# ahmetumutdurmus/zaremba

Measured on NVIDIA H100. Metric: tokens/sec (and valid perplexity) Large-LSTM 1500h at 1/2/4/8 H100 vs ref CPU, higher is better.
Workload: dtype f16 operands, f32 accumulate/state

## Files before the change

### zaremba_b200/csrc/gemm_tc.cu

```cuda
#include <stdlib.h>
#include <string.h>

#include "kernels.h"
#include "tc_common.cuh"
#include "tc_host.h"

namespace zrb {

using namespace tc;

constexpr int GBM = 128, GBK = 64;
constexpr int kASubBytes = GBM * GBK * 2;
constexpr int kEpiWarps = 8;
constexpr int kGemmThreads = 3 * 128;
template <int GBN> struct GemmCfg {
    static constexpr int kStages = GBN == 256 ? 4 : 6;
    static constexpr int kABytes = kASubBytes;
    static constexpr int kBBytes = GBN * GBK * 2;
    static constexpr int kSmem = kStages * (kABytes + kBBytes) + 1024  + 256 ;
};

struct GemmArgs {
    int M, N, K;
    float alpha;
    const float* bias;
    const float* bias2;
    float* C;
    int64_t ldc;
    int accumulate;
    int tiles_m, tiles_n;
    int splits;
    float* sumsq_out;
    float* C2;
    float* sumsq_out2;
    const __half* a_tiled;
    const __half* b_tiled;
    int a_nt128, b_nt128;
    int pdl_trigger;
    int pdl_tail;
    int epi_direct;
};

template <int GBN> constexpr int kStagger = GemmCfg<GBN>::kStages - 1;
constexpr int kStaggerBar = 1;

template <bool A_MN, bool B_MN, int GBN>
__global__ void __launch_bounds__(kGemmThreads, 1)
gemm_f16_tc_kernel(const __grid_constant__ CUtensorMap tma_a, const __grid_constant__ CUtensorMap tma_b,
                   const __grid_constant__ CUtensorMap tma_b2, GemmArgs p) {
    using Cfg = GemmCfg<GBN>;
    constexpr int kStages = Cfg::kStages;
    constexpr int kABytes = Cfg::kABytes;
    constexpr int kBBytes = Cfg::kBBytes;
    extern __shared__ uint8_t smem_raw[];
    uint8_t* smem = (uint8_t*)(((uintptr_t)smem_raw + 1023) & ~(uintptr_t)1023);
    uint8_t* sA = smem;
    uint8_t* sB = smem + kStages * kABytes;
    uint64_t* bars = (uint64_t*)(smem + kStages * (kABytes + kBBytes));
    uint64_t* full = bars;
    uint64_t* empty = bars + kStages;

    const int warp = __shfl_sync(0xffffffffu, (int)(threadIdx.x >> 5), 0);
    const int lane = threadIdx.x & 31;
    const int num_tiles = p.tiles_m * p.tiles_n;
    const int num_kb = (p.K + GBK - 1) / GBK;
    const bool dual = p.C2 != nullptr;
    const int num_work = dual ? 2 * num_tiles : num_tiles * p.splits;
    const int kb_per = (num_kb + p.splits - 1) / p.splits;

    if (threadIdx.x == 0) {
        if (p.pdl_trigger) asm volatile("griddepcontrol.launch_dependents;" ::: "memory");
        tma_prefetch_desc(&tma_a);
        tma_prefetch_desc(&tma_b);
        if (dual) tma_prefetch_desc(&tma_b2);
        for (int i = 0; i < kStages; ++i) { mbar_init(&full[i], 1); mbar_init(&empty[i], kEpiWarps); }
        fence_mbar_init();
    }
    __syncthreads();

    if (warp < 4) {
        asm volatile("setmaxnreg.dec.sync.aligned.u32 40;" ::: "memory");
        if (warp == 0 && lane == 0) {
            int s = 0; uint32_t ph = 0;
            for (int w = blockIdx.x; w < num_work; w += gridDim.x) {
                const int tile = w % num_tiles, sp = dual ? 0 : w / num_tiles;
                const int kb0 = sp * kb_per, kb1 = min(num_kb, kb0 + kb_per);
                const CUtensorMap* tmb = (dual && w >= num_tiles) ? &tma_b2 : &tma_b;
                const int m0 = (tile % p.tiles_m) * GBM, n0 = (tile / p.tiles_m) * GBN;
                for (int kb = kb0; kb < kb1; ++kb) {
                    mbar_wait(&empty[s], ph ^ 1);
                    mbar_expect_tx(&full[s], kABytes + kBBytes);
                    uint8_t* a = sA + s * kABytes;
                    uint8_t* b = sB + s * kBBytes;
                    if (!A_MN && p.a_tiled) {
                        bulk_load_1d(a, p.a_tiled + ((size_t)kb * p.a_nt128 + (m0 >> 7)) * (128 * GBK), kASubBytes, &full[s]);
                    } else if (!A_MN) {
                        tma_load_2d(a, &tma_a, &full[s], kb * GBK, m0);
                    } else {
                        tma_load_2d(a, &tma_a, &full[s], m0, kb * GBK);
                        tma_load_2d(a + kASubBytes / 2, &tma_a, &full[s], m0 + 64, kb * GBK);
                    }
                    if (!B_MN && p.b_tiled) {
                        bulk_load_1d(b, p.b_tiled + ((size_t)kb * p.b_nt128 + (n0 >> 7)) * (128 * GBK), kBBytes, &full[s]);
                    } else if (!B_MN) {
                        tma_load_2d(b, tmb, &full[s], kb * GBK, n0);
                    } else {
#pragma unroll
                        for (int j = 0; j < GBN / 64; ++j)
                            tma_load_2d(b + j * (GBK * 128), tmb, &full[s], n0 + 64 * j, kb * GBK);
                    }
                    if (++s == kStages) { s = 0; ph ^= 1; }
                }
            }
        }
    } else {
        asm volatile("setmaxnreg.inc.sync.aligned.u32 232;" ::: "memory");
        const int cw = warp - 4;
        const int wg = cw >> 2;
        const int t = (int)threadIdx.x - 128 * (1 + wg);
        int s = 0; uint32_t ph = 0;
        float acc[GBN / 2];
        bool started_wg1 = p.epi_direct || wg == 1;
        if (!p.epi_direct && wg == 1) asm volatile("bar.sync %0, 256;" :: "n"(kStaggerBar) : "memory");
        int kb_issued = 0;
        const bool pair_store = !p.epi_direct && !p.accumulate && (p.ldc & 1) == 0 && ((uintptr_t)p.C & 7) == 0 &&
                                ((uintptr_t)p.C2 & 7) == 0;
        for (int w = blockIdx.x; w < num_work; w += gridDim.x) {
            const int tile = w % num_tiles, split = dual ? 0 : w / num_tiles;
            const int kb0 = split * kb_per, kb1 = min(num_kb, kb0 + kb_per);
            float* const Cout = (dual && w >= num_tiles) ? p.C2 : p.C;
            float* const ssq = (dual && w >= num_tiles) ? p.sumsq_out2 : p.sumsq_out;
            const int m0 = (tile % p.tiles_m) * GBM + 64 * wg, n0 = (tile / p.tiles_m) * GBN;
#pragma unroll
            for (int i = 0; i < GBN / 2; ++i) acc[i] = 0.f;
            wgmma_fence();
            wgmma_fence_acc(acc);
            int prev = -1;
            for (int kb = kb0; kb < kb1; ++kb) {
                mbar_wait(&full[s], ph);
                const uint32_t a_addr = smem_u32(sA + s * kABytes) + wg * (kASubBytes / 2);
                const uint32_t b_addr = smem_u32(sB + s * kBBytes);
#pragma unroll
                for (int k = 0; k < GBK / 16; ++k) {
                    const uint64_t da = A_MN ? make_smem_desc(a_addr + k * 2048, GBK * 128, 1024, kSwizzle128B)
                                             : make_smem_desc(a_addr + k * 32, 16, 1024, kSwizzle128B);
                    const uint64_t db = B_MN ? make_smem_desc(b_addr + k * 2048, GBK * 128, 1024, kSwizzle128B)
                                             : make_smem_desc(b_addr + k * 32, 16, 1024, kSwizzle128B);
                    Wgmma<GBN, A_MN ? 1 : 0, B_MN ? 1 : 0>::mma(acc, da, db, 1u);
                }
                wgmma_commit();
                if (!started_wg1 && ++kb_issued == kStagger<GBN>) {
                    asm volatile("bar.arrive %0, 256;" :: "n"(kStaggerBar) : "memory");
                    started_wg1 = true;
                }
                wgmma_wait<1>();
                if (prev >= 0) {
                    __syncwarp();
                    if (lane == 0) mbar_arrive(&empty[prev]);
                }
                prev = s;
                if (++s == kStages) { s = 0; ph ^= 1; }
            }
            if (!started_wg1) {
                asm volatile("bar.arrive %0, 256;" :: "n"(kStaggerBar) : "memory");
                started_wg1 = true;
            }
            wgmma_wait<0>();
            wgmma_fence_acc(acc);
            if (prev >= 0) {
                __syncwarp();
                if (lane == 0) mbar_arrive(&empty[prev]);
            }
            const bool add_bias = p.bias != nullptr && split == 0;
            float ss = 0.f;
#pragma unroll
            for (int h = 0; h < 2; ++h) {
                const int row = m0 + wgmma_row(t, h);
                if (row >= p.M) continue;
                float* const crow = Cout + (int64_t)row * p.ldc;
#pragma unroll
                for (int c8 = 0; c8 < GBN / 8; ++c8) {
                    const int col0 = n0 + wgmma_col(t, c8);
                    if (pair_store && col0 + 1 < p.N) {
                        const float bv0 = add_bias ? p.bias[col0] + (p.bias2 ? p.bias2[col0] : 0.f) : 0.f;
                        const float bv1 = add_bias ? p.bias[col0 + 1] + (p.bias2 ? p.bias2[col0 + 1] : 0.f) : 0.f;
                        const float o0 = p.alpha * acc[4 * c8 + 2 * h] + bv0;
                        const float o1 = p.alpha * acc[4 * c8 + 2 * h + 1] + bv1;
                        if (p.splits > 1) {
                            atomicAdd(reinterpret_cast<float2*>(crow + col0), make_float2(o0, o1));
                        } else {
                            *reinterpret_cast<float2*>(crow + col0) = make_float2(o0, o1);
                            ss += o0 * o0;
                            ss += o1 * o1;
                        }
                        continue;
                    }
#pragma unroll
                    for (int e = 0; e < 2; ++e) {
                        const int col = n0 + wgmma_col(t, c8) + e;
                        if (col >= p.N) continue;
                        const float bv = add_bias ? p.bias[col] + (p.bias2 ? p.bias2[col] : 0.f) : 0.f;
                        const float o = p.alpha * acc[4 * c8 + 2 * h + e] + bv;
                        if (p.splits > 1) {
                            atomicAdd(crow + col, o);
                        } else if (p.accumulate) {
                            crow[col] += o;
                        } else {
                            crow[col] = o;
                            ss += o * o;
                        }
                    }
                }
            }
            if (ssq) {
                ss = warp_sum(ss);
                if (lane == 0) ssq[tile * 8 + cw] = ss;
            }
        }
        if (!started_wg1) asm volatile("bar.arrive %0, 256;" :: "n"(kStaggerBar) : "memory");
    }
    if (p.pdl_tail && blockIdx.x == 0 && threadIdx.x == 0) asm volatile("griddepcontrol.wait;" ::: "memory");
}

namespace {

typedef CUresult (*EncodeTiledFn)(CUtensorMap*, CUtensorMapDataType, cuuint32_t, void*, const cuuint64_t*,
                                  const cuuint64_t*, const cuuint32_t*, const cuuint32_t*, CUtensorMapInterleave,
                                  CUtensorMapSwizzle, CUtensorMapL2promotion, CUtensorMapFloatOOBfill);

EncodeTiledFn get_encode() {
    static EncodeTiledFn fn = nullptr;
    static bool tried = false;
    if (!tried) {
        tried = true;
        void* p = nullptr;
        cudaDriverEntryPointQueryResult q;
        if (cudaGetDriverEntryPoint("cuTensorMapEncodeTiled", &p, cudaEnableDefault, &q) == cudaSuccess &&
            q == cudaDriverEntryPointSuccess)
            fn = (EncodeTiledFn)p;
    }
    return fn;
}

int g_num_sms = 0;
bool g_attr_set[64][8] = {};

}

int tc_num_sms() {
    if (!g_num_sms) {
        int dev = 0;
        cudaGetDevice(&dev);
        cudaDeviceGetAttribute(&g_num_sms, cudaDevAttrMultiProcessorCount, dev);
        if (g_num_sms <= 0) g_num_sms = 132;
    }
    return g_num_sms;
}

int tc_make_tmap_f16(CUtensorMap* m, const void* ptr, uint64_t inner, uint64_t outer, uint64_t ld, uint32_t box_inner,
                     uint32_t box_outer, int swizzle128) {
    EncodeTiledFn enc = get_encode();
    if (!enc) {
        set_error("cuTensorMapEncodeTiled not available from the driver");
        return ZRB_E_CUDA;
    }
    ZRB_REQUIRE((ld * 2) % 16 == 0 && (((uintptr_t)ptr) & 15) == 0, "TMA operand needs 16-byte aligned base and pitch");
    cuuint64_t dims[2] = {inner, outer};
    cuuint64_t strides[1] = {ld * 2};
    cuuint32_t box[2] = {box_inner, box_outer};
    cuuint32_t estr[2] = {1, 1};
    CUresult r = enc(m, CU_TENSOR_MAP_DATA_TYPE_FLOAT16, 2, const_cast<void*>(ptr), dims, strides, box, estr,
                     CU_TENSOR_MAP_INTERLEAVE_NONE, swizzle128 ? CU_TENSOR_MAP_SWIZZLE_128B : CU_TENSOR_MAP_SWIZZLE_NONE,
                     CU_TENSOR_MAP_L2_PROMOTION_L2_256B, CU_TENSOR_MAP_FLOAT_OOB_FILL_NONE);
    if (r != CUDA_SUCCESS) {
        set_error("cuTensorMapEncodeTiled failed (%d) inner=%llu outer=%llu ld=%llu", (int)r,
                  (unsigned long long)inner, (unsigned long long)outer, (unsigned long long)ld);
        return ZRB_E_CUDA;
    }
    return ZRB_OK;
}

template <bool A_MN, bool B_MN, int GBN>
static int launch_gemm(const CUtensorMap& ta, const CUtensorMap& tb, const CUtensorMap& tb2, const GemmArgs& a,
                       cudaStream_t s) {
    auto kern = gemm_f16_tc_kernel<A_MN, B_MN, GBN>;
    const int idx = (A_MN ? 2 : 0) + (B_MN ? 1 : 0) + (GBN == 256 ? 4 : 0);
    int dev = 0;
    cudaGetDevice(&dev);
    dev &= 63;
    if (!g_attr_set[dev][idx]) {
        ZRB_CUDA(cudaFuncSetAttribute(kern, cudaFuncAttributeMaxDynamicSharedMemorySize, GemmCfg<GBN>::kSmem));
        g_attr_set[dev][idx] = true;
    }
    int grid = a.tiles_m * a.tiles_n * (a.C2 ? 2 : a.splits);
    if (grid > tc_num_sms()) grid = tc_num_sms();
    if (a.pdl_tail) {
        grid = a.tiles_m * a.tiles_n * (a.C2 ? 2 : a.splits);
        cudaLaunchConfig_t cfg = {};
        cfg.gridDim = dim3(grid); cfg.blockDim = dim3(kGemmThreads);
        cfg.dynamicSmemBytes = GemmCfg<GBN>::kSmem; cfg.stream = s;
        cudaLaunchAttribute at[1];
        at[0].id = cudaLaunchAttributeProgrammaticStreamSerialization;
        at[0].val.programmaticStreamSerializationAllowed = 1;
        cfg.attrs = at; cfg.numAttrs = 1;
        ZRB_CUDA(cudaLaunchKernelEx(&cfg, kern, ta, tb, tb2, a));
        count_launch();
        return ZRB_OK;
    }
    kern<<<grid, kGemmThreads, GemmCfg<GBN>::kSmem, s>>>(ta, tb, tb2, a);
    ZRB_KERNEL_CHECK();
    return ZRB_OK;
}

template <int GBN>
static int dispatch_gemm(const CUtensorMap& ta, const CUtensorMap& tb, const CUtensorMap& tb2, const GemmArgs& a,
                         int a_mn, int b_mn, cudaStream_t s) {
    if (!a_mn && !b_mn) return launch_gemm<false, false, GBN>(ta, tb, tb2, a, s);
    if (!a_mn && b_mn) return launch_gemm<false, true, GBN>(ta, tb, tb2, a, s);
    if (a_mn && !b_mn) return launch_gemm<true, false, GBN>(ta, tb, tb2, a, s);
    return launch_gemm<true, true, GBN>(ta, tb, tb2, a, s);
}

struct TileChoice { int bn, tiles_m, tiles_n, splits; };
static TileChoice choose_tiles(int M, int N, int num_kb, bool can_split, bool retile = false) {
    const int nsm = tc_num_sms();
    TileChoice c;
    c.tiles_m = cdiv(M, GBM);
    const int t256 = c.tiles_m * cdiv(N, 256);
    if (can_split && t256 * 2 <= nsm && t256 * 2 >= (nsm * 4) / 10 && num_kb / 2 >= 8) {
        c.bn = 256; c.tiles_n = cdiv(N, 256); c.splits = 2;
        return c;
    }
    c.bn = (t256 >= (nsm * 9) / 10) ? 256 : 128;
    static const int force_bn = [] { const char* e = getenv("ZRB_GEMM_BN"); return e ? atoi(e) : 0; }();
    if (force_bn == 128 || force_bn == 256) c.bn = force_bn;
    else if (retile && c.bn == 256 && cdiv(t256, nsm) * 2 > cdiv(c.tiles_m * cdiv(N, 128), nsm) &&
             c.tiles_m * cdiv(N, 128) * 2 > nsm)
        c.bn = 128;
    c.tiles_n = cdiv(N, c.bn);
    c.splits = (can_split && c.tiles_m * c.tiles_n * 2 <= nsm && num_kb >= 8) ? 2 : 1;
    return c;
}

int gemm_f16_tc_sumsq_slots(int M, int N, int K) {
    TileChoice c = choose_tiles(M, N, cdiv(K, GBK), false);
    return c.tiles_m * c.tiles_n * kEpiWarps;
}

int gemm_f16_tc(const __half* A, int64_t lda, int a_mn, const __half* B, int64_t ldb, int b_mn, float* C, int64_t ldc,
                int M, int N, int K, float alpha, const float* bias, int accumulate, cudaStream_t s, float* sumsq_out,
                const float* bias2, bool pdl, const __half* B2, float* C2, float* sumsq_out2, const __half* A_tiled,
                int a_nt128, const __half* B_tiled, int b_nt128) {
    if (M <= 0 || N <= 0) return ZRB_OK;
    ZRB_REQUIRE(!B2 == !C2, "dual launch needs both B2 and C2");
    ZRB_REQUIRE(!bias2 || bias, "bias2 needs bias");
    ZRB_REQUIRE(!sumsq_out || !accumulate, "sumsq_out needs a plain store epilogue");
    ZRB_REQUIRE(K > 0, "gemm_f16_tc needs K > 0");
    const char* epi = getenv("ZRB_GEMM_EPI");
    const bool direct = epi && strcmp(epi, "direct") == 0;
    const TileChoice tc = choose_tiles(M, N, cdiv(K, GBK), !sumsq_out && ldc == N && !C2 && !accumulate,
                                       !direct && !sumsq_out && !C2 && !accumulate);
    const int bn = tc.bn;
    CUtensorMap ta, tb;
    if (!a_mn) ZRB_TRY(tc_make_tmap_f16(&ta, A, K, M, lda, GBK, GBM, 1));
    else       ZRB_TRY(tc_make_tmap_f16(&ta, A, M, K, lda, 64, GBK, 1));
    if (!b_mn) ZRB_TRY(tc_make_tmap_f16(&tb, B, K, N, ldb, GBK, bn, 1));
    else       ZRB_TRY(tc_make_tmap_f16(&tb, B, N, K, ldb, 64, GBK, 1));
    CUtensorMap tb2 = tb;
    if (B2) {
        if (!b_mn) ZRB_TRY(tc_make_tmap_f16(&tb2, B2, K, N, ldb, GBK, bn, 1));
        else       ZRB_TRY(tc_make_tmap_f16(&tb2, B2, N, K, ldb, 64, GBK, 1));
    }
    GemmArgs a;
    a.M = M; a.N = N; a.K = K; a.alpha = alpha; a.bias = bias; a.C = C; a.ldc = ldc; a.accumulate = accumulate;
    a.tiles_m = tc.tiles_m; a.tiles_n = tc.tiles_n;
    a.splits = tc.splits;
    a.sumsq_out = sumsq_out;
    a.bias2 = bias2;
    a.C2 = C2; a.sumsq_out2 = sumsq_out2;
    a.a_tiled = a_mn ? nullptr : A_tiled; a.a_nt128 = a_nt128; a.b_tiled = b_mn ? nullptr : B_tiled; a.b_nt128 = b_nt128;
    a.pdl_tail = (pdl && a.splits == 1) ? 1 : 0;
    a.pdl_trigger = (rec_pdl_enabled() && !a.pdl_tail) ? 1 : 0;
    a.epi_direct = direct ? 1 : 0;
    if (a.splits > 1 && !accumulate) ZRB_CUDA(cudaMemsetAsync(C, 0, (size_t)M * N * sizeof(float), s));
    return bn == 256 ? dispatch_gemm<256>(ta, tb, tb2, a, a_mn, b_mn, s) : dispatch_gemm<128>(ta, tb, tb2, a, a_mn, b_mn, s);
}

}

extern "C" int zrb_gemm_f16_tiled(const void* A, int64_t lda, const void* B, int64_t ldb, const void* A_tiled, int32_t a_nt128,
                                  const void* B_tiled, int32_t b_nt128, float* C, int64_t ldc, int32_t M, int32_t N, int32_t K,
                                  float alpha, void* stream) {
    ZRB_REQUIRE(A && B && C, "null argument");
    return zrb::gemm_f16_tc((const __half*)A, lda, 0, (const __half*)B, ldb, 0, C, ldc, M, N, K, alpha, nullptr, 0,
                            (cudaStream_t)stream, nullptr, nullptr, false, nullptr, nullptr, nullptr, (const __half*)A_tiled,
                            a_nt128, (const __half*)B_tiled, b_nt128);
}

extern "C" int zrb_gemm_f16(const void* A, int64_t lda, int32_t a_mn_major, const void* B, int64_t ldb,
                            int32_t b_mn_major, float* C, int64_t ldc, int32_t M, int32_t N, int32_t K, float alpha,
                            const float* bias, int32_t accumulate, void* stream) {
    ZRB_REQUIRE(A && B && C, "null argument");
    return zrb::gemm_f16_tc((const __half*)A, lda, a_mn_major, (const __half*)B, ldb, b_mn_major, C, ldc, M, N, K,
                            alpha, bias, accumulate, (cudaStream_t)stream, nullptr, nullptr, false, nullptr, nullptr, nullptr, nullptr, 0, nullptr, 0);
}
```

Measured before the change: 385,500.

## Add ping-pong consumer warpgroup schedule for large 128x128 GEMMs

```diff
diff --git a/zaremba_b200/csrc/gemm_tc.cu b/zaremba_b200/csrc/gemm_tc.cu
--- a/zaremba_b200/csrc/gemm_tc.cu
+++ b/zaremba_b200/csrc/gemm_tc.cu
@@ -41,13 +41,69 @@
     int epi_direct;
 };
 
-template <int GBN> constexpr int kStagger = GemmCfg<GBN>::kStages - 1;
+template <int GBN> constexpr int kStagger = GBN == 256 ? 1 : 2;
 constexpr int kStaggerBar = 1;
-
-template <bool A_MN, bool B_MN, int GBN>
+constexpr int kTurnBar = 1;
+__device__ __forceinline__ void turn_sync(int g) {
+    if (g == 0) asm volatile("bar.sync %0, 256;" :: "n"(kTurnBar) : "memory");
+    else        asm volatile("bar.sync %0, 256;" :: "n"(kTurnBar + 1) : "memory");
+}
+__device__ __forceinline__ void turn_arrive(int g) {
+    if (g == 0) asm volatile("bar.arrive %0, 256;" :: "n"(kTurnBar) : "memory");
+    else        asm volatile("bar.arrive %0, 256;" :: "n"(kTurnBar + 1) : "memory");
+}
+
+template <int NC>
+__device__ __forceinline__ float store_rows(const GemmArgs& p, const float (&acc)[NC / 2], float* Cout, int m0, int n0,
+                                            int t, bool add_bias, bool pair_store) {
+    float ss = 0.f;
+#pragma unroll
+    for (int h = 0; h < 2; ++h) {
+        const int row = m0 + wgmma_row(t, h);
+        if (row >= p.M) continue;
+        float* const crow = Cout + (int64_t)row * p.ldc;
+#pragma unroll
+        for (int c8 = 0; c8 < NC / 8; ++c8) {
+            const int col0 = n0 + wgmma_col(t, c8);
+            if (pair_store && col0 + 1 < p.N) {
+                const float bv0 = add_bias ? p.bias[col0] + (p.bias2 ? p.bias2[col0] : 0.f) : 0.f;
+                const float bv1 = add_bias ? p.bias[col0 + 1] + (p.bias2 ? p.bias2[col0 + 1] : 0.f) : 0.f;
+                const float o0 = p.alpha * acc[4 * c8 + 2 * h] + bv0;
+                const float o1 = p.alpha * acc[4 * c8 + 2 * h + 1] + bv1;
+                if (p.splits > 1) {
+                    atomicAdd(reinterpret_cast<float2*>(crow + col0), make_float2(o0, o1));
+                } else {
+                    *reinterpret_cast<float2*>(crow + col0) = make_float2(o0, o1);
+                    ss += o0 * o0;
+                    ss += o1 * o1;
+                }
+                continue;
+            }
+#pragma unroll
+            for (int e = 0; e < 2; ++e) {
+                const int col = n0 + wgmma_col(t, c8) + e;
+                if (col >= p.N) continue;
+                const float bv = add_bias ? p.bias[col] + (p.bias2 ? p.bias2[col] : 0.f) : 0.f;
+                const float o = p.alpha * acc[4 * c8 + 2 * h + e] + bv;
+                if (p.splits > 1) {
+                    atomicAdd(crow + col, o);
+                } else if (p.accumulate) {
+                    crow[col] += o;
+                } else {
+                    crow[col] = o;
+                    ss += o * o;
+                }
+            }
+        }
+    }
+    return ss;
+}
+
+template <bool A_MN, bool B_MN, int GBN, bool PP>
 __global__ void __launch_bounds__(kGemmThreads, 1)
 gemm_f16_tc_kernel(const __grid_constant__ CUtensorMap tma_a, const __grid_constant__ CUtensorMap tma_b,
                    const __grid_constant__ CUtensorMap tma_b2, GemmArgs p) {
+    static_assert(!PP || GBN == 128, "ping-pong runs 128x128 tiles");
     using Cfg = GemmCfg<GBN>;
     constexpr int kStages = Cfg::kStages;
     constexpr int kABytes = Cfg::kABytes;
@@ -73,7 +129,7 @@
         tma_prefetch_desc(&tma_a);
         tma_prefetch_desc(&tma_b);
         if (dual) tma_prefetch_desc(&tma_b2);
-        for (int i = 0; i < kStages; ++i) { mbar_init(&full[i], 1); mbar_init(&empty[i], kEpiWarps); }
+        for (int i = 0; i < kStages; ++i) { mbar_init(&full[i], 1); mbar_init(&empty[i], PP ? kEpiWarps / 2 : kEpiWarps); }
         fence_mbar_init();
     }
     __syncthreads();
@@ -113,6 +169,70 @@
                 }
             }
         }
+    } else if constexpr (PP) {
+        asm volatile("setmaxnreg.inc.sync.aligned.u32 232;" ::: "memory");
+        const int wg = (warp - 4) >> 2;
+        const int t = (int)threadIdx.x - 128 * (1 + wg);
+        int s = 0; uint32_t ph = 0;
+        float acc[2][GBN / 2];
+        const bool pair_store = !p.accumulate && (p.ldc & 1) == 0 && ((uintptr_t)p.C & 7) == 0;
+        int j = 0;
+        for (int w = blockIdx.x; w < num_work; w += gridDim.x, ++j) {
+            const int tile = w % num_tiles, split = w / num_tiles;
+            const int kb0 = split * kb_per, kb1 = min(num_kb, kb0 + kb_per);
+            if ((j & 1) != wg) {
+                s += kb1 - kb0;
+                ph ^= (uint32_t)(s / kStages) & 1u;
+                s %= kStages;
+                continue;
+            }
+            if (j > 0) turn_sync(wg);
+            const int m0 = (tile % p.tiles_m) * GBM, n0 = (tile / p.tiles_m) * GBN;
+#pragma unroll
+            for (int r = 0; r < 2; ++r)
+#pragma unroll
+                for (int i = 0; i < GBN / 2; ++i) acc[r][i] = 0.f;
+            wgmma_fence();
+            wgmma_fence_acc(acc[0]);
+            wgmma_fence_acc(acc[1]);
+            int prev = -1;
+            for (int kb = kb0; kb < kb1; ++kb) {
+                mbar_wait(&full[s], ph);
+                const uint32_t a_addr = smem_u32(sA + s * kABytes);
+                const uint32_t b_addr = smem_u32(sB + s * kBBytes);
+#pragma unroll
+                for (int k = 0; k < GBK / 16; ++k) {
+                    const uint64_t db = B_MN ? make_smem_desc(b_addr + k * 2048, GBK * 128, 1024, kSwizzle128B)
+                                             : make_smem_desc(b_addr + k * 32, 16, 1024, kSwizzle128B);
+#pragma unroll
+                    for (int r = 0; r < 2; ++r) {
+                        const uint32_t ar = a_addr + r * (kASubBytes / 2);
+                        const uint64_t da = A_MN ? make_smem_desc(ar + k * 2048, GBK * 128, 1024, kSwizzle128B)
+                                                 : make_smem_desc(ar + k * 32, 16, 1024, kSwizzle128B);
+                        Wgmma<GBN, A_MN ? 1 : 0, B_MN ? 1 : 0>::mma(acc[r], da, db, 1u);
+                    }
+                }
+                wgmma_commit();
+                wgmma_wait<1>();
+                if (prev >= 0) {
+                    __syncwarp();
+                    if (lane == 0) mbar_arrive(&empty[prev]);
+                }
+                prev = s;
+                if (++s == kStages) { s = 0; ph ^= 1; }
+            }
+            if (w + (int)gridDim.x < num_work) turn_arrive(wg ^ 1);
+            wgmma_wait<0>();
+            wgmma_fence_acc(acc[0]);
+            wgmma_fence_acc(acc[1]);
+            if (prev >= 0) {
+                __syncwarp();
+                if (lane == 0) mbar_arrive(&empty[prev]);
+            }
+            const bool add_bias = p.bias != nullptr && split == 0;
+#pragma unroll
+            for (int r = 0; r < 2; ++r) store_rows<GBN>(p, acc[r], p.C, m0 + 64 * r, n0, t, add_bias, pair_store);
+        }
     } else {
         asm volatile("setmaxnreg.inc.sync.aligned.u32 232;" ::: "memory");
         const int cw = warp - 4;
@@ -172,46 +292,7 @@
                 if (lane == 0) mbar_arrive(&empty[prev]);
             }
             const bool add_bias = p.bias != nullptr && split == 0;
-            float ss = 0.f;
-#pragma unroll
-            for (int h = 0; h < 2; ++h) {
-                const int row = m0 + wgmma_row(t, h);
-                if (row >= p.M) continue;
-                float* const crow = Cout + (int64_t)row * p.ldc;
-#pragma unroll
-                for (int c8 = 0; c8 < GBN / 8; ++c8) {
-                    const int col0 = n0 + wgmma_col(t, c8);
-                    if (pair_store && col0 + 1 < p.N) {
-                        const float bv0 = add_bias ? p.bias[col0] + (p.bias2 ? p.bias2[col0] : 0.f) : 0.f;
-                        const float bv1 = add_bias ? p.bias[col0 + 1] + (p.bias2 ? p.bias2[col0 + 1] : 0.f) : 0.f;
-                        const float o0 = p.alpha * acc[4 * c8 + 2 * h] + bv0;
-                        const float o1 = p.alpha * acc[4 * c8 + 2 * h + 1] + bv1;
-                        if (p.splits > 1) {
-                            atomicAdd(reinterpret_cast<float2*>(crow + col0), make_float2(o0, o1));
-                        } else {
-                            *reinterpret_cast<float2*>(crow + col0) = make_float2(o0, o1);
-                            ss += o0 * o0;
-                            ss += o1 * o1;
-                        }
-                        continue;
-                    }
-#pragma unroll
-                    for (int e = 0; e < 2; ++e) {
-                        const int col = n0 + wgmma_col(t, c8) + e;
-                        if (col >= p.N) continue;
-                        const float bv = add_bias ? p.bias[col] + (p.bias2 ? p.bias2[col] : 0.f) : 0.f;
-                        const float o = p.alpha * acc[4 * c8 + 2 * h + e] + bv;
-                        if (p.splits > 1) {
-                            atomicAdd(crow + col, o);
-                        } else if (p.accumulate) {
-                            crow[col] += o;
-                        } else {
-                            crow[col] = o;
-                            ss += o * o;
-                        }
-                    }
-                }
-            }
+            float ss = store_rows<GBN>(p, acc, Cout, m0, n0, t, add_bias, pair_store);
             if (ssq) {
                 ss = warp_sum(ss);
                 if (lane == 0) ssq[tile * 8 + cw] = ss;
@@ -243,7 +324,7 @@
 }
 
 int g_num_sms = 0;
-bool g_attr_set[64][8] = {};
+bool g_attr_set[64][16] = {};
 
 }
 
@@ -280,11 +361,11 @@
     return ZRB_OK;
 }
 
-template <bool A_MN, bool B_MN, int GBN>
+template <bool A_MN, bool B_MN, int GBN, bool PP = false>
 static int launch_gemm(const CUtensorMap& ta, const CUtensorMap& tb, const CUtensorMap& tb2, const GemmArgs& a,
                        cudaStream_t s) {
-    auto kern = gemm_f16_tc_kernel<A_MN, B_MN, GBN>;
-    const int idx = (A_MN ? 2 : 0) + (B_MN ? 1 : 0) + (GBN == 256 ? 4 : 0);
+    auto kern = gemm_f16_tc_kernel<A_MN, B_MN, GBN, PP>;
+    const int idx = (A_MN ? 2 : 0) + (B_MN ? 1 : 0) + (GBN == 256 ? 4 : 0) + (PP ? 8 : 0);
     int dev = 0;
     cudaGetDevice(&dev);
     dev &= 63;
@@ -321,10 +402,11 @@
     return launch_gemm<true, true, GBN>(ta, tb, tb2, a, s);
 }
 
-struct TileChoice { int bn, tiles_m, tiles_n, splits; };
-static TileChoice choose_tiles(int M, int N, int num_kb, bool can_split, bool retile = false) {
+struct TileChoice { int bn, tiles_m, tiles_n, splits; bool pingpong; };
+static TileChoice choose_tiles_staggered(int M, int N, int num_kb, bool can_split, bool retile) {
     const int nsm = tc_num_sms();
     TileChoice c;
+    c.pingpong = false;
     c.tiles_m = cdiv(M, GBM);
     const int t256 = c.tiles_m * cdiv(N, 256);
     if (can_split && t256 * 2 <= nsm && t256 * 2 >= (nsm * 4) / 10 && num_kb / 2 >= 8) {
@@ -339,6 +421,16 @@
         c.bn = 128;
     c.tiles_n = cdiv(N, c.bn);
     c.splits = (can_split && c.tiles_m * c.tiles_n * 2 <= nsm && num_kb >= 8) ? 2 : 1;
+    return c;
+}
+static TileChoice choose_tiles(int M, int N, int num_kb, bool can_split, bool retile = false, bool pingpong_ok = false) {
+    TileChoice c = choose_tiles_staggered(M, N, num_kb, can_split, retile);
+    const int nsm = tc_num_sms(), items = c.tiles_m * cdiv(N, 128) * c.splits;
+    if (pingpong_ok && (items >= 3 * nsm || (c.splits == 2 && items >= nsm))) {
+        c.pingpong = true;
+        c.bn = 128;
+        c.tiles_n = cdiv(N, 128);
+    }
     return c;
 }
 
@@ -359,7 +451,8 @@
     const char* epi = getenv("ZRB_GEMM_EPI");
     const bool direct = epi && strcmp(epi, "direct") == 0;
     const TileChoice tc = choose_tiles(M, N, cdiv(K, GBK), !sumsq_out && ldc == N && !C2 && !accumulate,
-                                       !direct && !sumsq_out && !C2 && !accumulate);
+                                       !direct && !sumsq_out && !C2 && !accumulate,
+                                       !direct && !a_mn && !sumsq_out && !C2 && !pdl);
     const int bn = tc.bn;
     CUtensorMap ta, tb;
     if (!a_mn) ZRB_TRY(tc_make_tmap_f16(&ta, A, K, M, lda, GBK, GBM, 1));
@@ -383,6 +476,9 @@
     a.pdl_trigger = (rec_pdl_enabled() && !a.pdl_tail) ? 1 : 0;
     a.epi_direct = direct ? 1 : 0;
     if (a.splits > 1 && !accumulate) ZRB_CUDA(cudaMemsetAsync(C, 0, (size_t)M * N * sizeof(float), s));
+    if (tc.pingpong) {
+        return b_mn ? launch_gemm<false, true, 128, true>(ta, tb, tb2, a, s) : launch_gemm<false, false, 128, true>(ta, tb, tb2, a, s);
+    }
     return bn == 256 ? dispatch_gemm<256>(ta, tb, tb2, a, a_mn, b_mn, s) : dispatch_gemm<128>(ta, tb, tb2, a, a_mn, b_mn, s);
 }
 
```

Result: faster. 392,000, median of 6 (+1.7%).
